# dsteinberg/libcluster

Measured on AMD Instinct MI355X. Metric: E-step data-points/sec (full VBEM iteration: suff-stats + M-step + E-step), higher is better.
Workload: dtype f64

## Files before the change

libcluster_amd/csrc/lc_kernels.h:

```cpp
#pragma once
#include <hip/hip_runtime.h>
#include <cstdint>

namespace lck {

constexpr int RG = 16;

inline int padded_dim(int D) {
  return D <= 16 ? 16 : D <= 32 ? 32 : D <= 48 ? 48 : D <= 64 ? 64 : D <= 80 ? 80 : D <= 96 ? 96 : D <= 112 ? 112 : D <= 128 ? 128 : -1;
}
__host__ __device__ constexpr int lds_row_stride(int DP) { return DP == 16 ? 16 : (DP + 16) % 32 != 16 ? DP + 32 : DP + 16; }
inline int padded_dim_wide(int D) { return D <= 128 ? padded_dim(D) : (D + 63) / 64 * 64; }
constexpr int GW_MAX_DP = 1024;
inline int ntiles(int DP) { int nt = DP / 4; return nt * (nt + 1) / 2; }
inline int pstride(int DP) { return ntiles(DP) * 16 + DP; }
constexpr int WIDE_CHUNK = 256 * 16 + 64;
inline int wide_chunks(int DP) { int np = DP / 64; return np * (np + 1) / 2; }
inline int64_t estep_pstride(int DP, int DC) { return DP > 128 ? (int64_t)wide_chunks(DP) * WIDE_CHUNK : (int64_t)pstride(DC); }
inline int64_t estep_pstride(int DP) { return estep_pstride(DP, DP); }
inline int estep_active_width(int D, int DP) {
  if (DP < 32 || DP > 128) return DP;
  const int g = DP <= 48 ? 4 : 8, lo = DP <= 48 ? DP - 12 : DP - 8;
  const int dc = (D + g - 1) / g * g;
  return dc < DP ? (dc < lo ? lo : dc) : DP;
// ... 54 lines not shown
  int64_t nrg;
  const int* rginfo;
  int64_t nrows;
  const double* params;
  const double* ctab;
  int K;
  double* qZ;
  int64_t ldq;
  double* partial;
  bool want_ll;
  int grid;
  int ngroups = 1;
  int yshare = 0;
};
constexpr int FUSED_CT_CAP = 1024;
inline int64_t fused_record(int DP, int K) { return (int64_t)K * (1 + DP + (int64_t)DP * DP) + 1 + K; }
bool fused_eligible(int DP, int K);
int fused_plan(int DP, int64_t nrg, int K);
hipError_t launch_fused(const FusedLaunch& a, hipStream_t stream);

struct SSItem {
  int64_t r0, r1;
  int kofs, kcnt;
  int64_t rec0;
};
constexpr int SS_BR = 32;
constexpr double SPECK_TAU = 0x1p-300;
enum SuffstatRoute { SS_PER_CLUSTER = 0, SS_FEAT = 1, SS_QUAD = 2, SS_WIDE = 3 };
enum SuffstatMode { SS_DENSE = 0, SS_MASKED_DENSE = 1, SS_ZERO_SKIP = 2, SS_WORK_LIST = 3 };
struct SuffstatPlan {
  SuffstatRoute route;
  int nchunks;
  int64_t chunk_rows;
  int extra, klast0, KR;
  int clusters_per_block;
  const char* name;
};
SuffstatPlan suffstat_plan(int DP, int DC, int64_t NP, int K, SuffstatMode mode);
struct SuffstatLaunch {
  int DP;
  int DC = 0;
  const double* X;
  int64_t NP;
  const double* qZ;
  int64_t ldq;
  int K;
  SuffstatMode mode = SS_DENSE;
  const int* rginfo;
  const unsigned char* smask;
  double* partial;
  int nchunks = 0, KR = 0;
  int64_t chunk_rows = 0;
  const SSItem* items = nullptr;
  const int* klist = nullptr;
  int nitems = 0, skip_listed = 0;
  int speck_skip = 0;
  int nslice = 1;
  int slice0 = 0, rs = 1, klast0 = 0, nklast = 0;
  int64_t ldx = 0;
  int DPW = 0, colA = 0, colB = 0;
};
hipError_t launch_suffstat(const SuffstatLaunch& a, const SuffstatPlan& p, hipStream_t stream);

constexpr int SPECK_PROBE_STEPS = 4096;
constexpr int64_t SPECK_PROBE_MIN_ROWS = 4096;
hipError_t launch_speck_probe(const double* qZ, int64_t ldq, int K, int64_t NP, int* active, int64_t* pairs, hipStream_t stream,
                              int64_t* rows = nullptr);
inline bool speck_probe_says_skip(int64_t active, int64_t pairs) { return pairs > 0 && 4 * (pairs - active) >= pairs; }
bool speck_probe_says_lists(int64_t single, int64_t rows);

struct SsListLayout {
  int nq;
  bool wide;
  size_t ent_off;
  size_t bytes;
};
inline SsListLayout ss_list_layout(int nchunks, int64_t chunk_rows, int K) {
  SsListLayout l{(K + 3) / 4, chunk_rows > 65536, 0, 0};
  l.ent_off = ((size_t)nchunks * l.nq * sizeof(int) + 15) / 16 * 16;
  l.bytes = l.ent_off + (size_t)nchunks * l.nq * (size_t)chunk_rows * (l.wide ? 4 : 2);
  return l;
}
bool suffstat_list_instance(int DP, int DC);
bool speck_lists_enabled();
hipError_t launch_suffstat_list_build(const SuffstatLaunch& a, const SuffstatPlan& p, void* lists, size_t bytes, hipStream_t stream);
hipError_t launch_suffstat_lists(const SuffstatLaunch& a, const SuffstatPlan& p, void* lists, size_t bytes, hipStream_t stream);
hipError_t launch_suffstat_list_build_masks(const SuffstatLaunch& a, const SuffstatPlan& p, const unsigned short* qmask, int64_t nrg,
                                            void* lists, size_t bytes, hipStream_t stream);
hipError_t launch_suffstat_lists_masks(const SuffstatLaunch& a, const SuffstatPlan& p, const unsigned short* qmask, int64_t nrg,
                                       void* lists, size_t bytes, hipStream_t stream);
hipError_t launch_speck_probe_masks(const unsigned short* qmask, int64_t nrg, int K, int64_t NP, int* active, int64_t* pairs,
                                    hipStream_t stream, int64_t* rows = nullptr);
hipError_t launch_qmask_from_qz(const double* qZ, int64_t ldq, int K, int64_t nrg, unsigned short* qmask, hipStream_t stream);
int speck_skip_mode();

__host__ __device__ constexpr int ft_offdiag(int DC) { return (DC / 4) * (DC / 4 - 1) / 2; }
__host__ __device__ constexpr int ft_features(int DC) { return 16 * ft_offdiag(DC) + 10 * (DC / 4) + DC + 1; }
__host__ __device__ constexpr int ft_tiles(int DC) { return (ft_features(DC) + 15) / 16; }
enum FtKind { FT_PRODUCT = 0, FT_LINEAR = 1, FT_COUNT = 2, FT_SPARE = 3 };
struct FtFeature {
  int u, w, kind;
};
__host__ __device__ __attribute__((always_inline)) constexpr FtFeature ft_feature_rest(int DC, int one, int g) {
  const int ndiag = 10 * (DC / 4);
  if (g < ndiag) {
    const int b = 4 * (g / 10), e = g % 10;
    const int i = e < 4 ? 0 : e < 7 ? 1 : e < 9 ? 2 : 3, i0 = e < 4 ? 0 : e < 7 ? 4 : e < 9 ? 7 : 9;
    return {b + i, b + i + (e - i0), FT_PRODUCT};
  }
  g -= ndiag;
  if (g < DC) return {g, one, FT_LINEAR};
  return {one, one, g == DC ? FT_COUNT : FT_SPARE};
}
__host__ __device__ __attribute__((always_inline)) constexpr FtFeature ft_feature(int DC, int one, int f) {
  const int noff = 16 * ft_offdiag(DC);
  if (f < noff) {
    const int p = f / 16, r = f % 16;
    int ja = 1;
    while ((ja + 1) * ja / 2 <= p) ++ja;
    return {4 * (p - ja * (ja - 1) / 2) + (r & 3), 4 * ja + (r >> 2), FT_PRODUCT};
  }
  return ft_feature_rest(DC, one, f - noff);
}
#ifndef LC_FT_WAVES64
#define LC_FT_WAVES64 8
#endif
#ifndef LC_FT_WAVES128
#define LC_FT_WAVES128 8
#endif
__host__ __device__ constexpr int ft_waves(int DP) { return DP == 64 ? LC_FT_WAVES64 : DP == 128 ? LC_FT_WAVES128 : DP > 64 ? 8 : 4; }
__host__ __device__ constexpr int ft_tpw_max(int DP, int NQ) {
  const int t = (NQ >= 8 && DP > 64 && DP < 128 ? 64 : 72) / NQ;
  return t < 14 ? t : 14;
}
__host__ __device__ constexpr int ft_nslice(int DP, int DC, int NQ) {
  return (ft_tiles(DC) + ft_waves(DP) * ft_tpw_max(DP, NQ) - 1) / (ft_waves(DP) * ft_tpw_max(DP, NQ));
}
__host__ __device__ constexpr int ft_tpw(int DP, int DC, int NQ) {
  return (ft_tiles(DC) + ft_waves(DP) * ft_nslice(DP, DC, NQ) - 1) / (ft_waves(DP) * ft_nslice(DP, DC, NQ));
}
__host__ __device__ __attribute__((always_inline)) constexpr void ft_deal(int DP, int DC, int NQ, int slice, int wave, int* t0, int* nt) {
  const int tiles = ft_tiles(DC), nsl = ft_nslice(DP, DC, NQ);
  if (ft_waves(DP) == 8) {
    const int ns = 4 * nsl, s = slice * 4 + (wave & 3), l = tiles / ns, r = tiles % ns;
    const int load = l + (s < r ? 1 : 0), first = s * l + (s < r ? s : r);
    *t0 = first + (wave < 4 ? 0 : (load + 1) / 2);
    *nt = wave < 4 ? (load + 1) / 2 : load / 2;
  } else {
    const int tpw = ft_tpw(DP, DC, NQ), t = (slice * 4 + wave) * tpw;
    *t0 = t;
    *nt = tiles - t < tpw ? (tiles - t > 0 ? tiles - t : 0) : tpw;
  }
}
__host__ __device__ constexpr int ftl_tpw(int DC) { return ((ft_tiles(DC) + 3) / 4 + 1) / 2; }
__host__ __device__ __attribute__((always_inline)) constexpr void ft_deal_one(int DC, int wave, int* t0, int* nt) {
  const int tiles = ft_tiles(DC), s = wave & 3, l = tiles / 4, r = tiles % 4;
  const int load = l + (s < r ? 1 : 0), first = s * l + (s < r ? s : r);
  *t0 = first + (wave < 4 ? 0 : (load + 1) / 2);
  *nt = wave < 4 ? (load + 1) / 2 : load / 2;
}
#ifndef LC_FTL_SHARED
#define LC_FTL_SHARED 1
#endif
__host__ __device__ constexpr bool ftl_shared(int DC) { return LC_FTL_SHARED != 0 && DC == 64; }
__host__ __device__ constexpr int ftl_paired(int DC) { return ftl_shared(DC) ? DC / 4 - 1 : 0; }
__host__ __device__ constexpr int ftl_split(int DC) { return ftl_shared(DC) ? DC / 8 : 0; }
struct FtlFeature {
  int u, w, kind;
  int shared;
};
__host__ __device__ __attribute__((always_inline)) constexpr FtlFeature ftl_feature(int DC, int one, int wave, int t, int l16) {
  if (!ftl_shared(DC)) {
    int t0 = 0, nt = 0;
    ft_deal_one(DC, wave, &t0, &nt);
    if (t >= nt) return {one, one, FT_SPARE, -1};
    const FtFeature f = ft_feature(DC, one, 16 * (t0 + t) + l16);
    return {f.u, f.w, f.kind, -1};
  }
  const int nb = DC / 4, S = ftl_split(DC), P = ftl_paired(DC);
  if (t < P) {
    const int second = t >= S ? 1 : 0, a = wave + second * S, o = (a + 1 + t - second * S) % nb;
    return {4 * o + (l16 & 3), 4 * a + (l16 >> 2), FT_PRODUCT, second};
  }
  const FtFeature f = ft_feature_rest(DC, one, 16 * (2 * wave + t - P) + l16);
  return {f.u, f.w, f.kind, -1};
}
__host__ __device__ constexpr int ftl_nw(int DC) { return ftl_shared(DC) ? 2 + ftl_tpw(DC) - ftl_paired(DC) : ftl_tpw(DC); }
__host__ __device__ constexpr int ftl_wi(int DC, int t) {
  return !ftl_shared(DC) ? t : t < ftl_split(DC) ? 0 : t < ftl_paired(DC) ? 1 : 2 + t - ftl_paired(DC);
}
static_assert(!ftl_shared(64) || (ftl_tpw(64) == ftl_paired(64) + 2 && 16 * 2 * 8 >= ft_features(64) - 16 * ft_offdiag(64)),
              "shared deal: 8 waves of two stars and two free tiles");

__host__ __device__ constexpr int ft_nt_min(int DP, int DC, int NQ) {
  int m = ft_tpw(DP, DC, NQ);
  for (int sl = 0; sl < ft_nslice(DP, DC, NQ); ++sl)
    for (int w = 0; w < ft_waves(DP); ++w) {
      int t0 = 0, nt = 0;
      ft_deal(DP, DC, NQ, sl, w, &t0, &nt);
      m = nt < m ? nt : m;
    }
  return m;
}

hipError_t launch_fold_extra(double* rec, int64_t SS, int K, int klast0, int extra, hipStream_t stream);
hipError_t launch_reduce_records(const double* partial, int64_t n, int K, const int* kptr, const int* krec, double* out,
                                 hipStream_t stream);

constexpr int REDUCE_TMP_ELEMS = 512;
hipError_t launch_reduce_partials(const double* partial, int nparts, int64_t n, double* out, hipStream_t stream,
                                  double* tmp = nullptr);
hipError_t launch_group_colsum(const double* qZ, int64_t ldq, int K, const int64_t* goff, int J, double* out,
                               hipStream_t stream, double* tmp = nullptr, int64_t rows = 0);
hipError_t launch_fill_qz(double* qZ, int64_t ldq, int K, const int* rginfo, int64_t nrows, int64_t nrg, double value,
                          hipStream_t stream);
struct DiagEstepLaunch {
  int DP, D;
  const double* X;
  int64_t nrg;
  const int* rginfo;
  int64_t nrows;
  const double* params;
  int mode = 0;
  const double* ctab;
  int K;
  double* qZ;
  int64_t ldq;
  double* fz_part;
  double* ll_part;
  int raw = 0;
  const double* wt = nullptr;
  const double* mu = nullptr;
  const double* constk = nullptr;
  int ngroups = 1;
  double* sink = nullptr;
};
constexpr int EDM_CT_CAP = 1024;
inline int64_t estep_diag_grid(int64_t nrg) { return (nrg * RG + 63) / 64; }
int64_t estep_diag_mfma_weights(int DP, int K, int mode);
enum DiagEstepInstance { EDI_NONE = 0, EDI_GENERIC = 1, EDI_PLAIN = 2, EDI_TABLED = 3, EDI_ONEGROUP = 4 };
struct DiagEstepPlan {
  bool ok;
  bool mfma;
  int mode;
  int64_t grid;
  size_t lds_bytes;
  const char* name;
  bool wide;
  int KT;
  bool REG;
  int NT;
  bool QUAD;
  int R, KTM;
  int instance;
  int64_t nslots;
  int per_cu;
  int64_t block_cap;
};
DiagEstepPlan estep_diag_plan(const DiagEstepLaunch& a);
hipError_t launch_estep_diag(const DiagEstepLaunch& a, hipStream_t stream);
double estep_diag_centre(int D, int DP, int K, int mode, const double* a, const double* w2, double* mu);
void estep_diag_pack(int D, int DP, int K, int mode, const double* a, const double* w2, const double* w1, const double* mu,
                     double* constk, double* wt, int64_t nw);

struct DiagStatLaunch {
  int DP;
  const double* X;
  int64_t NP;
  const double* qZ;
  int64_t ldq;
  int K;
  const int* rginfo;
  const unsigned char* smask;
  double* partial;
  int nchunks;
// ... 209 lines not shown
```

libcluster_amd/csrc/lc_kernels_suffstat.hip:

```cpp
#include "lc_device.hpp"

#ifndef LC_SS_FEAT_MINK_ACTIVE
#define LC_SS_FEAT_MINK_ACTIVE 5
#endif
#ifndef LC_SS_FEAT_WIDTHS
#define LC_SS_FEAT_WIDTHS(DP) ((DP) >= 32 && (DP) <= 128)
#endif

namespace lck {

template <int NB>
struct SSAcc { static constexpr int N = NB * 3 + NB * (NB - 1) / 2 * 4; };

template <int NB>
__host__ __device__ constexpr bool ss_in_half(int half, int jbp, int jb) {
  if (half == 0) return true;
  const bool first = NB == 8   ? (jbp < 5 || (jbp == 5 && jb < 3))
                     : NB == 7 ? (jbp < 4 || (jbp == 4 && jb < 4))
                     : NB == 6 ? (jbp < 4 || (jbp == 4 && jb < 1))
                               : (jbp == 1 || jbp == 2);
  return first == (half == 1);
}
template <int PAN>
constexpr int ss_batch_rows() { return PAN == 2 ? 24 : SS_BR; }
// ... 1191 lines not shown
#pragma unroll
        for (int t = 0; t < NT; ++t) acc[t] = mfma4(qc, pp[t], acc[t]);
        __builtin_amdgcn_sched_barrier(0);
      } else {
        __builtin_amdgcn_sched_barrier(0);
#pragma unroll
        for (int t = 0; t < NT; ++t) {
          acc[t] = mfma4(qc, pp[t], acc[t]);
          if (st + 1 < BR / 4 && t < SPREAD) {
#pragma unroll
            for (int r = t * NRD / SPREAD; r < (t + 1) * NRD / SPREAD; ++r) {
              const int what = ftl_read(DC, r);
              if (what == NT)
                qa = pq[QO + (st + 1) * 4 * QLD];
              else if (what >= 0)
                uf[what] = pu[what][XO + (st + 1) * 4 * LD];
              else
                wf[-1 - what] = pw[-1 - what][XO + (st + 1) * 4 * LD];
            }
          }
          __builtin_amdgcn_sched_barrier(0);
        }
      }
    }
  };
  if constexpr (LATE) {
    for (int p0 = 0; p0 < len; p0 += 2 * BR) {
      gload();
      iload(p0 + 2 * BR);
      batch(std::integral_constant<int, 0>{});
      lstore(1);
      __syncthreads();
      if (p0 + BR >= len) break;
      gload();
      iload(p0 + 3 * BR);
      batch(std::integral_constant<int, 1>{});
      lstore(0);
      __syncthreads();
    }
  } else {
    for (int p0 = 0; p0 < len; p0 += 2 * BR) {
      const bool more1 = p0 + BR < len, more2 = p0 + 2 * BR < len;
      if (more1) {
        gload();
        iload(p0 + 2 * BR);
      }
      batch(std::integral_constant<int, 0>{});
      if (more1) lstore(1);
      __syncthreads();
      if (!more1) break;
      if (more2) {
        gload();
        iload(p0 + 3 * BR);
      }
      batch(std::integral_constant<int, 1>{});
      if (more2) lstore(0);
      __syncthreads();
    }
  }

  const int64_t SS = 1 + (int64_t)DP + (int64_t)DP * DP;
  int wv = wave;
  asm volatile("" : "+v"(wv));
  const int kk = 4 * quad + hi;
  if (kk >= a.K) return;
  double* out = a.partial + ((int64_t)chunk * a.KR + kk) * SS;
#pragma unroll
  for (int t = 0; t < NT; ++t) {
    const FtlFeature f = ftl_feature(DC, ONE, wv, t, lo2 + 4 * blk);
    if (f.kind == FT_SPARE) continue;
    const double v = acc[t];
    if (f.kind == FT_PRODUCT) {
      double* S = out + 1 + DP;
      S[(int64_t)f.u * DP + f.w] = v;
      S[(int64_t)f.w * DP + f.u] = v;
    } else if (f.kind == FT_LINEAR) {
      out[1 + f.u] = v;
    } else {
      out[0] = v;
    }
  }
}

static hipError_t ss_list_check(const SuffstatLaunch& a, const SuffstatPlan& p, const void* lists, size_t bytes, SsListLayout* lay) {
  if (a.K <= 0 || p.nchunks <= 0 || !lists || !a.qZ || !a.X) return hipErrorInvalidValue;
  if (p.route != SS_FEAT || a.mode != SS_DENSE || a.smask || a.items || p.extra != 0) return hipErrorInvalidValue;
  if (a.nchunks != p.nchunks || a.chunk_rows != p.chunk_rows || a.KR != p.KR || a.KR != a.K) return hipErrorInvalidValue;
  if (!suffstat_list_instance(a.DP, a.DC)) return hipErrorInvalidValue;
  if (a.chunk_rows < 4 || a.chunk_rows % 4 || a.chunk_rows > (int64_t)1 << 30 || (int64_t)a.nchunks * a.chunk_rows < a.NP) return hipErrorInvalidValue;
  *lay = ss_list_layout(a.nchunks, a.chunk_rows, a.K);
  if ((int64_t)a.nchunks * lay->nq > (int64_t)1 << 30 || bytes < lay->bytes) return hipErrorInvalidValue;
  return hipSuccess;
}
hipError_t launch_suffstat_list_build(const SuffstatLaunch& a, const SuffstatPlan& p, void* lists, size_t bytes, hipStream_t stream) {
  SsListLayout lay;
  if (hipError_t e = ss_list_check(a, p, lists, bytes, &lay); e != hipSuccess) return e;
  int* lens = static_cast<int*>(lists);
  void* ent = static_cast<char*>(lists) + lay.ent_off;
  if (lay.wide)
    hipLaunchKernelGGL(ss_list_build_kernel<unsigned>, dim3((unsigned)a.nchunks), dim3(256), 0, stream, a.qZ, a.ldq, a.K, a.NP,
                       a.chunk_rows, lay.nq, lens, static_cast<unsigned*>(ent));
  else
    hipLaunchKernelGGL(ss_list_build_kernel<unsigned short>, dim3((unsigned)a.nchunks), dim3(256), 0, stream, a.qZ, a.ldq, a.K, a.NP,
                       a.chunk_rows, lay.nq, lens, static_cast<unsigned short*>(ent));
  return hipGetLastError();
}
template <int DP, int DC, typename IT>
static hipError_t launch_ss_list_i(const SuffstatLaunch& a, const SsListLayout& lay, const void* lists, hipStream_t stream) {
  constexpr int BR = LC_FTL_BR;
  const size_t shmem = (size_t)(2 * BR * lds_row_stride(DP) + 2 * BR * 4) * sizeof(double);
  auto kern = suffstat_list_kernel<DP, DC, IT>;
  static LdsGrant grant;
  if (hipError_t e = grant_dynamic_lds(reinterpret_cast<const void*>(kern), shmem, grant); e != hipSuccess) return e;
  hipLaunchKernelGGL(kern, dim3((unsigned)(a.nchunks * lay.nq)), dim3(512), shmem, stream, a, static_cast<const int*>(lists),
                     reinterpret_cast<const IT*>(static_cast<const char*>(lists) + lay.ent_off), lay.nq);
  return hipGetLastError();
}
hipError_t launch_suffstat_lists(const SuffstatLaunch& a, const SuffstatPlan& p, void* lists, size_t bytes, hipStream_t stream) {
  SsListLayout lay;
  if (hipError_t e = ss_list_check(a, p, lists, bytes, &lay); e != hipSuccess) return e;
  if (hipError_t e = launch_suffstat_list_build(a, p, lists, bytes, stream); e != hipSuccess) return e;
  const bool narrow = a.DC == 56;
  if (lay.wide) return narrow ? launch_ss_list_i<64, 56, unsigned>(a, lay, lists, stream) : launch_ss_list_i<64, 64, unsigned>(a, lay, lists, stream);
  return narrow ? launch_ss_list_i<64, 56, unsigned short>(a, lay, lists, stream)
                : launch_ss_list_i<64, 64, unsigned short>(a, lay, lists, stream);
}

template <typename IT>
__global__ void __launch_bounds__(256) ss_list_build_masks_kernel(const unsigned short* __restrict__ qmask, int64_t nrg, int64_t NP,
                                                                   int64_t chunk_rows, int nq, int* __restrict__ lens, IT* __restrict__ ent) {
  __shared__ int wcnt[2][4];
  const int chunk = blockIdx.x / nq, c = blockIdx.x % nq, tid = threadIdx.x, lane = tid & 63, wave = tid >> 6;
  const int64_t r0 = (int64_t)chunk * chunk_rows;
  const int64_t r1 = (r0 + chunk_rows) < NP ? (r0 + chunk_rows) : NP;
  if (r0 >= r1) {
    if (tid == 0) lens[blockIdx.x] = 0;
    return;
  }
  const unsigned short* mq = qmask + (int64_t)c * nrg;
  IT* seg = ent + (int64_t)blockIdx.x * chunk_rows;
  int base = 0, par = 0;
  for (int64_t t0 = r0; t0 < r1; t0 += 4096, par ^= 1) {
    const int64_t row = t0 + 16 * tid;
    unsigned m = 0;
    if (row < r1) {
      const int64_t w = row >> 4;
      const unsigned sh = (unsigned)(row & 15);
      const unsigned lo = mq[w], hi = sh != 0 && w + 1 < nrg ? mq[w + 1] : 0u;
      m = ((lo | (hi << 16)) >> sh) & 0xffffu;
      if (r1 - row < 16) m &= (1u << (unsigned)(r1 - row)) - 1u;
    }
    const int cnt = __popc(m);
    int inc = cnt;
#pragma unroll
    for (int d = 1; d < 64; d <<= 1) {
      const int up = __shfl_up(inc, d);
      if (lane >= d) inc += up;
    }
    if (lane == 63) wcnt[par][wave] = inc;
    __syncthreads();
    int before = 0, tot = 0;
#pragma unroll
    for (int w = 0; w < 4; ++w) {
      const int n = wcnt[par][w];
      before += w < wave ? n : 0;
      tot += n;
    }
    int at = base + before + inc - cnt;
    while (m) {
      const int i = __ffs((int)m) - 1;
      m &= m - 1;
      seg[at++] = (IT)(row - r0 + i);
    }
    base += tot;
  }
  if (tid == 0) lens[blockIdx.x] = base;
}
__global__ void __launch_bounds__(256) qmask_from_qz_kernel(const double* __restrict__ qZ, int64_t ldq, int K, int64_t nrg,
                                                             unsigned short* __restrict__ qmask) {
  const int64_t row = (int64_t)blockIdx.x * 256 + threadIdx.x;
  const int c = blockIdx.y, lane = threadIdx.x & 63;
  bool keep = false;
  if (row < nrg * RG) {
#pragma unroll
    for (int i = 0; i < 4; ++i) {
      const int k = 4 * c + i;
      if (k < K && speck_keeps(qZ[(int64_t)k * ldq + row])) keep = true;
    }
  }
  const unsigned long long b = __ballot(keep);
  if ((lane & 15) == 0 && row < nrg * RG) qmask[(int64_t)c * nrg + (row >> 4)] = (unsigned short)((b >> lane) & 0xffffull);
}
hipError_t launch_qmask_from_qz(const double* qZ, int64_t ldq, int K, int64_t nrg, unsigned short* qmask, hipStream_t stream) {
  if (!qZ || !qmask || K < 1 || nrg < 1 || ldq < nrg * RG || (K + 3) / 4 > 65535) return hipErrorInvalidValue;
  hipLaunchKernelGGL(qmask_from_qz_kernel, dim3((unsigned)((nrg * RG + 255) / 256), (unsigned)((K + 3) / 4)), dim3(256), 0, stream, qZ, ldq,
                     K, nrg, qmask);
  return hipGetLastError();
}
hipError_t launch_suffstat_list_build_masks(const SuffstatLaunch& a, const SuffstatPlan& p, const unsigned short* qmask, int64_t nrg,
                                            void* lists, size_t bytes, hipStream_t stream) {
  SsListLayout lay;
  if (hipError_t e = ss_list_check(a, p, lists, bytes, &lay); e != hipSuccess) return e;
  if (!qmask || nrg * RG < a.NP) return hipErrorInvalidValue;
  int* lens = static_cast<int*>(lists);
  void* ent = static_cast<char*>(lists) + lay.ent_off;
  const dim3 grid((unsigned)(a.nchunks * lay.nq));
  if (lay.wide)
    hipLaunchKernelGGL(ss_list_build_masks_kernel<unsigned>, grid, dim3(256), 0, stream, qmask, nrg, a.NP, a.chunk_rows, lay.nq, lens,
                       static_cast<unsigned*>(ent));
  else
    hipLaunchKernelGGL(ss_list_build_masks_kernel<unsigned short>, grid, dim3(256), 0, stream, qmask, nrg, a.NP, a.chunk_rows, lay.nq, lens,
                       static_cast<unsigned short*>(ent));
  return hipGetLastError();
}
hipError_t launch_suffstat_lists_masks(const SuffstatLaunch& a, const SuffstatPlan& p, const unsigned short* qmask, int64_t nrg,
                                       void* lists, size_t bytes, hipStream_t stream) {
  SsListLayout lay;
  if (hipError_t e = launch_suffstat_list_build_masks(a, p, qmask, nrg, lists, bytes, stream); e != hipSuccess) return e;
  if (hipError_t e = ss_list_check(a, p, lists, bytes, &lay); e != hipSuccess) return e;
  const bool narrow = a.DC == 56;
  if (lay.wide) return narrow ? launch_ss_list_i<64, 56, unsigned>(a, lay, lists, stream) : launch_ss_list_i<64, 64, unsigned>(a, lay, lists, stream);
  return narrow ? launch_ss_list_i<64, 56, unsigned short>(a, lay, lists, stream)
                : launch_ss_list_i<64, 64, unsigned short>(a, lay, lists, stream);
}

struct SqItem {
  int kind, ia, ja;
};
__host__ __device__ constexpr int sq_items(int DC) { return (DC / 4) * (DC / 4 + 1) / 2 + DC / 4 + 1; }
__host__ __device__ constexpr SqItem sq_item(int DC, int n) {
  for (int ja = 0; ja < DC / 4; ++ja) {
    if (n <= ja) return SqItem{0, n, ja};
    n -= ja + 1;
    if (n == 0) return SqItem{1, 0, ja};
    n -= 1;
  }
  return SqItem{2, 0, 0};
}
__host__ __device__ constexpr int sq_part_lo(int DC, int NPART, int p) { return (sq_items(DC) * p + NPART - 1) / NPART; }
__host__ __device__ constexpr int sq_part_max(int DC, int NPART) {
  int m = 0;
  for (int p = 0; p < NPART; ++p) {
    const int n = sq_part_lo(DC, NPART, p + 1) - sq_part_lo(DC, NPART, p);
    m = n > m ? n : m;
  }
  return m;
}
constexpr int SQ_BR = 32, SQ_QLD = 18;
inline int sq_npart(int DP, int K) {
  const int nq = (K + 3) / 4;
  if (DP > 48) return 4;
  return nq == 2 ? 2 : nq == 4 ? (DP <= 32 ? 1 : 2) : 4;
}
inline int sq_nslice(int DP, int K) { return (((K + 3) / 4) * sq_npart(DP, K) + 3) / 4; }
inline bool ss_quad_eligible(int DP, int K) {
  static const int mode = test_switch("LC_SS_QUAD") ? atoi(test_switch("LC_SS_QUAD")) : -1;
  if (mode == 0 || DP < 32 || DP > 64 || K < 1 || K > 16) return false;
  if (mode == 1) return true;
  return K >= 3;
}
template <int DP, int DC, int NPART>
__global__ void __launch_bounds__(256, 2) suffstat_quad_kernel(SuffstatLaunch a) {
  static_assert(DC % 4 == 0 && DC <= DP && DC > DP - 16, "active width");
  constexpr int NT = DC / 4, BR = SQ_BR, LD = lds_row_stride(DP), QLD = SQ_QLD, XBUF = BR * LD, QBUF = BR * QLD, NTHR = 256;
  constexpr int NACC = sq_part_max(DC, NPART);
  extern __shared__ __attribute__((aligned(16))) double lds[];
  double* xbuf = lds;
  double* qbuf = lds + 2 * XBUF;
  const int tid = threadIdx.x, lane = tid & 63, wave = tid >> 6;
  const int hi = lane >> 4, blk = (lane >> 2) & 3, lo2 = lane & 3;
  const int K = a.K, NQ = (K + 3) / 4;
  int chunk, slice;
  {
    const int nslice = a.nslice, nchunks = a.nchunks, b = blockIdx.x, full = (nchunks / 8) * 8;
    if (b < full * nslice) {
      const int xcd = b & 7, seq = b >> 3;
      chunk = (seq / nslice) * 8 + xcd;
      slice = seq % nslice;
    } else {
      const int t = b - full * nslice;
      chunk = full + t / nslice;
      slice = t % nslice;
    }
  }
  const int64_t r0 = (int64_t)chunk * a.chunk_rows;
  const int64_t r1 = (r0 + a.chunk_rows) < a.NP ? (r0 + a.chunk_rows) : a.NP;
  const int unit = slice * 4 + wave, quad = unit / NPART, part = unit % NPART;
  const bool busy = quad < NQ;

  constexpr int TPR = DP / 2, NV2 = BR * TPR, NPRE = (NV2 + NTHR - 1) / NTHR;
  double pre[NPRE][2], qpre[4];
  const int qcl = tid % 16, qrq = tid / 16;
  const bool qthr = qrq < BR / 4;
  auto gload = [&](int64_t b0) {
#pragma unroll
    for (int i = 0; i < NPRE; ++i) {
      const int idx = tid + i * NTHR;
      const int row = idx / TPR, c2 = idx % TPR;
      double2 v = make_double2(0.0, 0.0);
      if (row < BR && b0 + row < r1) v = *reinterpret_cast<const double2*>(a.X + (b0 + row) * DP + 2 * c2);
      pre[i][0] = v.x;
      pre[i][1] = v.y;
    }
    const int64_t qrow = b0 + 4 * qrq;
#pragma unroll
    for (int i = 0; i < 4; ++i) qpre[i] = 0.0;
// ... 400 lines not shown
```

libcluster_amd/csrc/lc_testhooks.hip:

```cpp
#include <algorithm>
#include <cstdio>
#include <vector>

#include "lc_device.hpp"
#include "lc_predict.hpp"

namespace {

using lck::RG;
typedef long long i64;

class Scope {
 public:
  ~Scope() {
    for (auto& b : bufs_)
      if (b.d) (void)hipFree(b.d);
  }
  template <typename T>
  T* in(const T* h, size_t n) { return static_cast<T*>(add(const_cast<T*>(h), n * sizeof(T), false, true)); }
  template <typename T>
  T* io(T* h, size_t n) { return static_cast<T*>(add(h, n * sizeof(T), true, true)); }
  template <typename T>
  T* out(T* h, size_t n) { return static_cast<T*>(add(h, n * sizeof(T), true, false)); }
  template <typename T>
// ... 656 lines not shown
      if (klist[t] < 0 || klist[t] >= K) return -1;
    std::vector<char> used((size_t)nrec, 0);
    std::vector<std::vector<int>> recs((size_t)K);
    for (int i = 0; i < nitems; ++i) {
      if (r0[i] < 0 || r0[i] > r1[i] || r1[i] > NP || r0[i] % RG || r1[i] % RG) return -1;
      if (kcnt[i] < 1 || kcnt[i] > p.clusters_per_block || kofs[i] < 0 || kofs[i] > nklist - kcnt[i]) return -1;
      if (rec0[i] < 0 || rec0[i] > nrec - kcnt[i]) return -1;
      for (int t = 0; t < kcnt[i]; ++t) {
        if (used[(size_t)(rec0[i] + t)]) return -1;
        used[(size_t)(rec0[i] + t)] = 1;
        recs[(size_t)klist[kofs[i] + t]].push_back((int)(rec0[i] + t));
      }
      items.push_back(lck::SSItem{r0[i], r1[i], kofs[i], kcnt[i], rec0[i]});
    }
    kptr.assign((size_t)K + 1, 0);
    for (int k = 0; k < K; ++k) {
      krec.insert(krec.end(), recs[(size_t)k].begin(), recs[(size_t)k].end());
      kptr[(size_t)k + 1] = (int)krec.size();
    }
  }
  if (npartial < nrec * SS) return -1;
  Scope s;
  lck::SuffstatLaunch a{};
  a.DP = DP;
  a.DC = DC;
  a.X = s.in(X, (size_t)NP * DP);
  a.NP = NP;
  a.qZ = s.in(qZ, (size_t)K * (size_t)ldq);
  a.ldq = ldq;
  a.K = K;
  a.mode = m;
  a.rginfo = masked ? s.in(rginfo, (size_t)(NP / RG)) : nullptr;
  a.smask = masked ? s.in(smask, (size_t)J * K) : nullptr;
  a.partial = s.io(partial, (size_t)npartial);
  a.nchunks = p.nchunks;
  a.KR = p.KR;
  a.chunk_rows = p.chunk_rows;
  a.speck_skip = speck_skip < 0 ? (p.route == lck::SS_FEAT ? lck::speck_skip_mode() : 0) : speck_skip;
  const int* dkptr = nullptr;
  const int* dkrec = nullptr;
  if (listed) {
    a.items = s.in(items.data(), items.size());
    a.klist = s.in(klist, (size_t)nklist);
    a.nitems = nitems;
    a.skip_listed = skip_listed ? 1 : 0;
    if (fold) {
      dkptr = s.in(kptr.data(), kptr.size());
      dkrec = s.in(krec.data(), krec.size());
    }
  }
  double* dfold = fold ? s.io(folded, (size_t)nfolded) : nullptr;
  double* ext = fold && !listed && p.extra > 0 ? s.scratch<double>((size_t)p.KR * (size_t)SS) : nullptr;
  if (!s.ok()) return s.finish(hipSuccess);
  hipError_t e = lck::launch_suffstat(a, p, nullptr);
  if (e == hipSuccess && fold) {
    if (listed) {
      e = lck::launch_reduce_records(a.partial, SS, K, dkptr, dkrec, dfold, nullptr);
    } else if (p.extra > 0) {
      e = lck::launch_reduce_partials(a.partial, p.nchunks, (i64)p.KR * SS, ext, nullptr);
      if (e == hipSuccess) e = lck::launch_fold_extra(ext, SS, K, p.klast0, p.extra, nullptr);
      if (e == hipSuccess) e = hipMemcpyAsync(dfold, ext, (size_t)K * (size_t)SS * sizeof(double), hipMemcpyDeviceToDevice, nullptr);
    } else {
      e = lck::launch_reduce_partials(a.partial, p.nchunks, (i64)K * SS, dfold, nullptr);
    }
  }
  return s.finish(e);
}
LC_HOOK lc_test_suffstat(const double* X, int DP, int DC, i64 NP, const double* qZ, int K, i64 ldq, int mode, const int* rginfo,
                         const unsigned char* smask, int J, int nitems, const i64* r0, const i64* r1, const int* kofs, const int* kcnt,
                         const i64* rec0, const int* klist, int nklist, int nrec_listed, int skip_listed, double* partial, i64 npartial,
                         int fold, double* folded, i64 nfolded, i64* plan_out) {
  return test_suffstat(X, DP, DC, NP, qZ, K, ldq, mode, rginfo, smask, J, nitems, r0, r1, kofs, kcnt, rec0, klist, nklist, nrec_listed,
                       skip_listed, partial, npartial, fold, folded, nfolded, plan_out, -1);
}
LC_HOOK lcx_test_suffstat_speck(const double* X, int DP, int DC, i64 NP, const double* qZ, int K, i64 ldq, int mode, const int* rginfo,
                                const unsigned char* smask, int J, int nitems, const i64* r0, const i64* r1, const int* kofs,
                                const int* kcnt, const i64* rec0, const int* klist, int nklist, int nrec_listed, int skip_listed,
                               double* partial, i64 npartial, int fold, double* folded, i64 nfolded, i64* plan_out, int speck_skip) {
  if (speck_skip < 0 || speck_skip > 2) return -1;
  return test_suffstat(X, DP, DC, NP, qZ, K, ldq, mode, rginfo, smask, J, nitems, r0, r1, kofs, kcnt, rec0, klist, nklist, nrec_listed,
                       skip_listed, partial, npartial, fold, folded, nfolded, plan_out, speck_skip);
}

LC_HOOK lcx_test_suffstat_lists(const double* X, int DP, int DC, i64 NP, const double* qZ, int K, i64 ldq, int sums, double* partial,
                                i64 npartial, int fold, double* folded, i64 nfolded, i64* plan_out, int* lens_out, i64 nlens, int* ent_out,
                                i64 nent) {
  if (!X || !qZ || !partial || !plan_out || !lens_out || !ent_out || K < 1 || K > 4096 || !gw_width_ok(DP, DC)) return -1;
  if (NP < RG || NP % RG || NP > HOT_MAX_NRG * RG || ldq < NP || ldq % 2) return -1;
  const i64 SS = lck::stat_stride(DP);
  if (fold && (!sums || !folded || nfolded < (i64)K * SS)) return -1;
  const lck::SuffstatPlan p = lck::suffstat_plan(DP, DC, NP, K, lck::SS_DENSE);
  plan_out[0] = p.route, plan_out[1] = p.nchunks, plan_out[2] = p.chunk_rows, plan_out[3] = p.extra, plan_out[4] = p.klast0;
  plan_out[5] = p.KR, plan_out[6] = p.clusters_per_block;
  if (p.nchunks < 1 || p.chunk_rows < lck::SS_BR || p.chunk_rows % lck::SS_BR || (i64)p.nchunks * p.chunk_rows < NP) return -1;
  const lck::SsListLayout lay = lck::ss_list_layout(p.nchunks, p.chunk_rows, K);
  const i64 nseg = (i64)p.nchunks * lay.nq;
  if (npartial < (i64)p.nchunks * p.KR * SS || nlens < nseg || nent < nseg * p.chunk_rows) return -1;
  Scope s;
  lck::SuffstatLaunch a{};
  a.DP = DP;
  a.DC = DC;
  a.X = s.in(X, (size_t)NP * DP);
  a.NP = NP;
  a.qZ = s.in(qZ, (size_t)K * (size_t)ldq);
  a.ldq = ldq;
  a.K = K;
  a.mode = lck::SS_DENSE;
  a.rginfo = nullptr;
  a.smask = nullptr;
  a.partial = s.io(partial, (size_t)npartial);
  a.nchunks = p.nchunks;
  a.KR = p.KR;
  a.chunk_rows = p.chunk_rows;
  unsigned char* lists = s.scratch<unsigned char>(lay.bytes);
  double* dfold = fold ? s.io(folded, (size_t)nfolded) : nullptr;
  if (!s.ok()) return s.finish(hipSuccess);
  hipError_t e = hipMemset(lists, 0xff, lay.bytes);
  if (e == hipSuccess)
    e = sums ? lck::launch_suffstat_lists(a, p, lists, lay.bytes, nullptr) : lck::launch_suffstat_list_build(a, p, lists, lay.bytes, nullptr);
  if (e == hipSuccess && fold) e = lck::launch_reduce_partials(a.partial, p.nchunks, (i64)K * SS, dfold, nullptr);
  const int rc = s.finish(e);
  if (rc != 0) return rc;
  std::vector<unsigned char> raw(lay.bytes);
  if (hipMemcpy(raw.data(), lists, lay.bytes, hipMemcpyDeviceToHost) != hipSuccess) return -1;
  const int* lens = reinterpret_cast<const int*>(raw.data());
  for (i64 g = 0; g < nseg; ++g)
    if (lens[g] < 0 || lens[g] > p.chunk_rows) return -2;
  for (i64 g = 0; g < nseg; ++g) {
    lens_out[g] = lens[g];
    for (int i = 0; i < lens[g]; ++i) {
      const size_t at = (size_t)g * (size_t)p.chunk_rows + (size_t)i;
      ent_out[at] = lay.wide ? (int)reinterpret_cast<const unsigned*>(raw.data() + lay.ent_off)[at]
                             : (int)reinterpret_cast<const unsigned short*>(raw.data() + lay.ent_off)[at];
    }
  }
  return 0;
}

LC_HOOK lcx_test_estep_masks(const double* X, int DP, int DC, i64 nrg, const double* params, const double* ctab, int J, const int* rginfo,
                             i64 nrows, int K, double* qZ, int Kbuf, i64 ldq, double* fz_part, i64 nfz, double* ll_part, i64 nll,
                             unsigned short* qmask, i64 nmask, int* emits) {
  if (!X || !params || !ctab || !qZ || !fz_part || !emits || K < 1 || K > 4096 || Kbuf < K || Kbuf > 8192 || J < 1 || J > (1 << 20)) return -1;
  if (nrg < 1 || nrg > HOT_MAX_NRG || ldq < nrg * RG || !gw_width_ok(DP, DC)) return -1;
  if (rginfo ? !rginfo_ok(rginfo, nrg, J) : (J != 1 || nrows < 0 || nrows > nrg * RG)) return -1;
  if (qmask && nmask < (i64)((K + 3) / 4) * nrg) return -1;
  lck::EstepLaunch a{};
  a.DP = DP;
  a.DC = DC;
  a.K = K;
  a.nrg = nrg;
  a.nrows = nrows;
  a.ldq = ldq;
  const lck::EstepPlan p = lck::estep_plan(a);
  if (!p.ok || p.grid < 1 || p.lds_bytes > HOT_LDS_LIMIT) return -1;
  if (nfz < p.grid || (ll_part && nll < p.grid * K)) return -1;
  *emits = p.emits ? 1 : 0;
  Scope s;
  a.X = s.in(X, (size_t)(nrg * RG) * DP);
  a.params = s.in(params, (size_t)K * (size_t)lck::estep_pstride(DP, p.DC));
  a.ctab = s.in(ctab, (size_t)J * K);
  a.rginfo = rginfo ? s.in(rginfo, (size_t)nrg) : nullptr;
  a.qZ = s.io(qZ, (size_t)Kbuf * (size_t)ldq);
  a.fz_part = s.io(fz_part, (size_t)nfz);
  a.ll_part = ll_part ? s.io(ll_part, (size_t)nll) : nullptr;
  a.qmask = qmask ? s.io(qmask, (size_t)nmask) : nullptr;
  if (!s.ok()) return s.finish(hipSuccess);
  return s.finish(lck::launch_estep(a, nullptr));
}

LC_HOOK lcx_test_list_build(int which, const double* qZ, int DC, i64 NP, int K, i64 ldq, const unsigned short* qmask, i64 chunk_rows,
                            i64* out, int* lens_out, i64 nlens, int* ent_out, i64 nent) {
  const int DP = 64;
  if (!qZ || !qmask || !out || !lens_out || !ent_out || K < 1 || K > 4096 || !gw_width_ok(DP, DC)) return -1;
  if (NP < RG || NP % RG || NP > HOT_MAX_NRG * RG || ldq < NP || chunk_rows < 0 || chunk_rows % 4) return -1;
  lck::SuffstatPlan p = lck::suffstat_plan(DP, DC, NP, K, lck::SS_DENSE);
  if (chunk_rows > 0) {
    p.chunk_rows = chunk_rows;
    p.nchunks = (int)((NP + chunk_rows - 1) / chunk_rows);
  }
  if (p.nchunks < 1 || p.chunk_rows < 4 || (i64)p.nchunks * p.chunk_rows < NP) return -1;
  out[0] = p.nchunks, out[1] = p.chunk_rows;
  const lck::SsListLayout lay = lck::ss_list_layout(p.nchunks, p.chunk_rows, K);
  const i64 nseg = (i64)p.nchunks * lay.nq, nrg = NP / RG;
  if (nlens < nseg || nent < nseg * p.chunk_rows) return -1;
  Scope s;
  lck::SuffstatLaunch a{};
  a.DP = DP;
  a.DC = DC;
  a.X = s.scratch<double>(16);
  a.NP = NP;
  a.qZ = s.in(qZ, (size_t)K * (size_t)ldq);
  a.ldq = ldq;
  a.K = K;
  a.mode = lck::SS_DENSE;
  a.nchunks = p.nchunks;
  a.KR = p.KR;
  a.chunk_rows = p.chunk_rows;
  const unsigned short* dmask = s.in(qmask, (size_t)lay.nq * (size_t)nrg);
  unsigned char* lists = s.scratch<unsigned char>(lay.bytes);
  if (!s.ok()) return s.finish(hipSuccess);
  hipError_t e = hipMemset(lists, 0xff, lay.bytes);
  if (e == hipSuccess)
    e = which ? lck::launch_suffstat_list_build_masks(a, p, dmask, nrg, lists, lay.bytes, nullptr)
              : lck::launch_suffstat_list_build(a, p, lists, lay.bytes, nullptr);
  const int rc = s.finish(e);
  if (rc != 0) return rc;
  std::vector<unsigned char> raw(lay.bytes);
  if (hipMemcpy(raw.data(), lists, lay.bytes, hipMemcpyDeviceToHost) != hipSuccess) return -1;
  const int* lens = reinterpret_cast<const int*>(raw.data());
  for (i64 g = 0; g < nseg; ++g)
    if (lens[g] < 0 || lens[g] > p.chunk_rows) return -2;
  for (i64 g = 0; g < nseg; ++g) {
    lens_out[g] = lens[g];
    for (int i = 0; i < lens[g]; ++i) {
      const size_t at = (size_t)g * (size_t)p.chunk_rows + (size_t)i;
      ent_out[at] = lay.wide ? (int)reinterpret_cast<const unsigned*>(raw.data() + lay.ent_off)[at]
                             : (int)reinterpret_cast<const unsigned short*>(raw.data() + lay.ent_off)[at];
    }
  }
  return 0;
}

LC_HOOK lcx_test_speck_probe(int which, const double* qZ, i64 ldq, int K, i64 NP, const unsigned short* qmask, i64* out) {
  if (!qZ || !qmask || !out || K < 1 || K > 4096 || NP < RG || NP % RG || NP > HOT_MAX_NRG * RG || ldq < NP || ldq % 2) return -1;
  const i64 nrg = NP / RG;
  Scope s;
  const double* dq = s.in(qZ, (size_t)K * (size_t)ldq);
  const unsigned short* dm = s.in(qmask, (size_t)((K + 3) / 4) * (size_t)nrg);
  int* act = s.scratch<int>(2);
  if (!s.ok()) return s.finish(hipSuccess);
  int64_t pairs = 0, rows = 0;
  const hipError_t e = which ? lck::launch_speck_probe_masks(dm, nrg, K, NP, act, &pairs, nullptr, &rows)
                             : lck::launch_speck_probe(dq, ldq, K, NP, act, &pairs, nullptr, &rows);
  const int rc = s.finish(e);
  if (rc != 0) return rc;
  int h[2] = {0, 0};
  if (hipMemcpy(h, act, sizeof(h), hipMemcpyDeviceToHost) != hipSuccess) return -1;
  out[0] = h[0], out[1] = h[1], out[2] = pairs, out[3] = rows;
  return 0;
}

LC_HOOK lcx_test_suffstat_list_deal(int DP, int DC, i64* info, int* feat, i64 nfeat) {
  if (!info || !feat || !gw_width_ok(DP, DC) || !lck::suffstat_list_instance(DP, DC)) return -1;
  const int dc = DC ? DC : DP, waves = 8, tiles = lck::ftl_tpw(dc);
  if (nfeat < (i64)waves * tiles * 16 * 4) return -1;
  info[0] = lck::ftl_shared(dc) ? 1 : 0, info[1] = waves, info[2] = tiles, info[3] = lck::ftl_paired(dc), info[4] = lck::ftl_split(dc);
  info[5] = DP;
  for (int v = 0; v < waves; ++v)
    for (int t = 0; t < tiles; ++t)
      for (int l = 0; l < 16; ++l) {
        const lck::FtlFeature f = lck::ftl_feature(dc, DP, v, t, l);
        int* o = feat + ((size_t)(v * tiles + t) * 16 + l) * 4;
        o[0] = f.u, o[1] = f.w, o[2] = f.kind, o[3] = f.shared;
      }
  return 0;
}

LC_HOOK lc_test_fused_plan(int DP, i64 nrg, int K, i64* out) {
  if (!out || K < 1 || K > 4096 || nrg < 0 || nrg > HOT_MAX_NRG || DP < 1 || DP > 1024) return -1;
  out[0] = lck::fused_eligible(DP, K) ? 1 : 0;
  out[1] = lck::fused_plan(DP, nrg, K);
  out[2] = lck::current_device_cus();
  out[3] = (i64)lck::fused_record(DP, K);
  return 0;
}
LC_HOOK lc_test_fused(const double* X, int D, i64 nrg, const double* params, const double* ctab, int J, const int* rginfo, i64 nrows,
                      int K, int want_ll, int grid, double* qZ, int Kbuf, i64 ldq, double* partial, i64 npartial, int* grid_used) {
  const int DP = 16;
  if (!X || !params || !ctab || !qZ || !partial || !grid_used || D < 1 || D > DP || K < 1 || Kbuf < K || Kbuf > 8192) return -1;
  if (nrg < 1 || nrg > HOT_MAX_NRG || ldq < nrg * RG || J < 1 || J > (1 << 20) || !lck::fused_eligible(DP, K)) return -1;
  if (rginfo ? !rginfo_ok(rginfo, nrg, J) : (J != 1 || nrows < 0 || nrows > nrg * RG)) return -1;
  const int plan = lck::fused_plan(DP, nrg, K);
  if (plan < 1 || grid < 0 || grid > plan) return -1;
  const int g = grid ? grid : plan;
  if (npartial < (i64)g * lck::fused_record(DP, K)) return -1;
  *grid_used = g;
  Scope s;
  lck::FusedLaunch a{};
  a.DP = DP;
  a.D = D;
  a.X = s.in(X, (size_t)(nrg * RG) * DP);
  a.nrg = nrg;
  a.rginfo = rginfo ? s.in(rginfo, (size_t)nrg) : nullptr;
  a.nrows = nrows;
  a.params = s.in(params, (size_t)K * (size_t)lck::pstride(DP));
  a.ctab = s.in(ctab, (size_t)J * K);
  a.K = K;
  a.qZ = s.io(qZ, (size_t)Kbuf * (size_t)ldq);
  a.ldq = ldq;
  a.partial = s.io(partial, (size_t)npartial);
  a.want_ll = want_ll != 0;
  a.grid = g;
  a.ngroups = J;
  if (!s.ok()) return s.finish(hipSuccess);
  return s.finish(lck::launch_fused(a, nullptr));
}

namespace {

bool diag_width_ok(int DP) { return DP >= 16 && (DP <= 128 ? DP % 16 == 0 : (DP % 64 == 0 && DP <= 1024)); }

void diag_estep_plan_out(const lck::DiagEstepPlan& p, i64* out, char* name) {
  out[0] = p.ok ? 1 : 0, out[1] = p.mfma ? 1 : 0, out[2] = p.mode, out[3] = p.grid, out[4] = (i64)p.lds_bytes;
  out[5] = p.wide ? 1 : 0, out[6] = p.KT, out[7] = p.REG ? 1 : 0, out[8] = p.NT, out[9] = p.QUAD ? 1 : 0, out[10] = p.R;
  out[11] = p.KTM, out[12] = p.instance, out[13] = p.nslots, out[14] = p.per_cu, out[15] = p.block_cap;
  if (name) snprintf(name, 32, "%s", p.name ? p.name : "");
}
void diag_stat_plan_out(const lck::DiagStatPlan& p, i64* out, char* name) {
  out[0] = p.ok ? 1 : 0, out[1] = p.nslice, out[2] = p.rsplit, out[3] = p.second, out[4] = p.nblocks, out[5] = p.width;
  out[6] = p.last_width, out[7] = p.BR, out[8] = p.BR_last, out[9] = p.nstage ? 1 : 0, out[10] = p.nstage_last ? 1 : 0;
  out[11] = p.deep ? 1 : 0, out[12] = p.deep_last ? 1 : 0, out[13] = (i64)p.lds_bytes;
  if (name) snprintf(name, 32, "%s", p.name ? p.name : "");
}
constexpr int DIAG_SINK = 256, DIAG_SINK_GUARD = 64;

}

LC_HOOK lc_test_estep_diag_plan(int DP, int K, int mode, i64 nrg, int mfma, int raw, int want_ll, int grouped, int ngroups,
                                i64* out, char* name) {
  if (!out || !name || K < 1 || K > 4096 || nrg < 0 || nrg > HOT_MAX_NRG || DP < 1 || DP > 1024 || mode < 0 || mode > 2 || ngroups < 1)
    return -1;
  static double some;
  static int somei;
  lck::DiagEstepLaunch a{};
  a.DP = DP, a.D = DP, a.K = K, a.mode = mode, a.nrg = nrg, a.raw = raw ? 1 : 0, a.ngroups = ngroups;
  a.wt = mfma ? &some : nullptr;
  a.ll_part = want_ll ? &some : nullptr;
  a.rginfo = grouped ? &somei : nullptr;
  diag_estep_plan_out(lck::estep_diag_plan(a), out, name);
  return 0;
}
LC_HOOK lc_test_estep_diag(const double* X, int DP, i64 nrg, const double* params, int mode, const double* ctab, int J,
                           const int* rginfo, i64 nrows, int K, int raw, const double* wt, i64 nwt, const double* mu,
                           const double* constk, double* qZ, int Kbuf, i64 ldq, double* fz_part, i64 nfz, double* ll_part, i64 nll,
                           double* sink, i64* plan_out, char* name) {
  if (!X || !params || !ctab || !qZ || !fz_part || !plan_out || !name || K < 1 || K > 4096 || Kbuf < K || Kbuf > 8192) return -1;
  if (J < 1 || J > (1 << 20) || mode < 0 || mode > 2 || nrg < 1 || nrg > HOT_MAX_NRG || nrg * RG > ldq) return -1;
  if (!diag_width_ok(DP)) return -1;
  if (rginfo ? !rginfo_ok(rginfo, nrg, J) : (J != 1 || nrows < 0 || nrows > nrg * RG)) return -1;
  if (wt) {
// ... 90 lines not shown
```

Measured before the change: 392.3 million.

## Add column-owner suffstat kernel for DP=64 list path

Adds a new sufficient-statistics kernel for D=64 on the sparse list route. Each cluster gets one wave, and each lane owns a column, accumulating 33 cyclic diagonals of the outer product in registers. Row values are broadcast through LDS and several rows are prefetched in flight, replacing the previous tile-dealt feature kernel. The aim is fewer wasted accumulators and better reuse, at the cost of more per-row LDS round trips and wave barriers, plus mirrored writes for the symmetric output.

Result: faster. 417.1 million (median of 6 runs) (+6.3%).

```diff
diff --git a/libcluster_amd/csrc/lc_kernels.h b/libcluster_amd/csrc/lc_kernels.h
--- a/libcluster_amd/csrc/lc_kernels.h
+++ b/libcluster_amd/csrc/lc_kernels.h
@@ -160,6 +160,7 @@
   return l;
 }
 bool suffstat_list_instance(int DP, int DC);
+bool suffstat_owner_instance(int DP, int DC);
 bool speck_lists_enabled();
 hipError_t launch_suffstat_list_build(const SuffstatLaunch& a, const SuffstatPlan& p, void* lists, size_t bytes, hipStream_t stream);
 hipError_t launch_suffstat_lists(const SuffstatLaunch& a, const SuffstatPlan& p, void* lists, size_t bytes, hipStream_t stream);
@@ -269,6 +270,13 @@
 }
 static_assert(!ftl_shared(64) || (ftl_tpw(64) == ftl_paired(64) + 2 && 16 * 2 * 8 >= ft_features(64) - 16 * ft_offdiag(64)),
               "shared deal: 8 waves of two stars and two free tiles");
+
+constexpr int FTO_DIAGS = 33, FTO_ACCS = 35;
+__host__ __device__ __attribute__((always_inline)) constexpr FtFeature fto_feature(int lane, int t) {
+  if (t < FTO_DIAGS) return {lane, (lane + t) & 63, t == 32 && lane >= 32 ? FT_SPARE : FT_PRODUCT};
+  if (t == FTO_DIAGS) return {lane, 64, FT_LINEAR};
+  return {64, 64, lane == 0 ? FT_COUNT : FT_SPARE};
+}
 
 __host__ __device__ constexpr int ft_nt_min(int DP, int DC, int NQ) {
   int m = ft_tpw(DP, DC, NQ);
diff --git a/libcluster_amd/csrc/lc_kernels_suffstat.hip b/libcluster_amd/csrc/lc_kernels_suffstat.hip
--- a/libcluster_amd/csrc/lc_kernels_suffstat.hip
+++ b/libcluster_amd/csrc/lc_kernels_suffstat.hip
@@ -1297,6 +1297,137 @@
   }
 }
 
+#ifndef LC_FTL_OWNER
+#define LC_FTL_OWNER 1
+#endif
+#ifndef LC_FTO_DEPTH
+#define LC_FTO_DEPTH 4
+#endif
+#ifndef LC_FTO_FUSED
+#define LC_FTO_FUSED 1
+#endif
+bool suffstat_owner_instance(int DP, int DC) { return LC_FTL_OWNER != 0 && DP == 64 && (DC == 0 || DC == 64); }
+template <int DP, int DC, typename IT>
+__global__ void __launch_bounds__(256, 4) suffstat_owner_kernel(SuffstatLaunch a, const int* __restrict__ lens, const IT* __restrict__ ent,
+                                                                 int nq) {
+  static_assert(DP == 64 && DC == 64, "lane w owns column w");
+  constexpr int G = LC_FTO_DEPTH, NSLOT = 2, ND = FTO_DIAGS;
+  static_assert(G >= 1 && G <= 8, "rows in flight");
+  __shared__ double slots[4][NSLOT][2 * DP];
+  const int lane = threadIdx.x & 63, wave = __builtin_amdgcn_readfirstlane((int)(threadIdx.x >> 6));
+  const int chunk = blockIdx.x / nq, quad = blockIdx.x % nq;
+  const int k = 4 * quad + wave;
+  if (k >= a.K) return;
+  const int64_t r0 = (int64_t)chunk * a.chunk_rows;
+  const int64_t rows64 = a.NP - r0 < a.chunk_rows ? a.NP - r0 : a.chunk_rows;
+  const int rows = rows64 > 0 ? (int)rows64 : 0;
+  int len = lens[blockIdx.x];
+  len = len < 0 ? 0 : len > rows ? rows : len;
+  const int nwin = (len + 63) / 64;
+  const IT* li = ent + (int64_t)blockIdx.x * a.chunk_rows;
+  const int64_t rb = rows > 0 ? r0 : 0;
+  const double* qcol = a.qZ + (int64_t)k * a.ldq + rb;
+  const double* xl = a.X + rb * DP + lane;
+  double* slot = &slots[wave][0][lane];
+
+  double acc[ND], lin = 0.0, cnt = 0.0;
+#pragma unroll
+  for (int t = 0; t < ND; ++t) acc[t] = 0.0;
+
+  auto ld_off = [&](int w) {
+    const int p = 64 * w + lane;
+    const int o = p < len ? (int)li[p] : 0;
+    return o < rows ? o : 0;
+  };
+  int widx = -1;
+  unsigned long long mask = 0ull;
+  int cur_off = 0, n1_off = ld_off(0), n2_off = ld_off(1);
+  double cur_q = 0.0, n1_q = qcol[n1_off];
+  auto advance = [&]() {
+    ++widx;
+    cur_off = n1_off, cur_q = n1_q;
+    n1_off = n2_off;
+    n1_q = qcol[n1_off];
+    n2_off = ld_off(widx + 2);
+    mask = __ballot(64 * widx + lane < len && speck_keeps(cur_q));
+  };
+  auto fetch = [&](double(&gx)[G], double(&gq)[G], int& n) {
+    while (mask == 0ull && widx + 1 < nwin) advance();
+    n = 0;
+#pragma unroll
+    for (int i = 0; i < G; ++i) {
+      const bool has = mask != 0ull;
+      const int l = has ? __builtin_ctzll(mask) : 0;
+      mask &= mask - (has ? 1ull : 0ull);
+      const int off = has ? __builtin_amdgcn_readlane(cur_off, l) : 0;
+      gq[i] = readlane_f64(cur_q, l);
+      gx[i] = xl[(int64_t)off * DP];
+      n += has ? 1 : 0;
+    }
+  };
+  auto row = [&](double x, double q, int s) {
+    double* sl = slot + s * 2 * DP;
+    __builtin_amdgcn_fence(__ATOMIC_RELEASE, "wavefront");
+    __builtin_amdgcn_wave_barrier();
+    sl[0] = x;
+    sl[DP] = x;
+    __builtin_amdgcn_fence(__ATOMIC_ACQ_REL, "wavefront");
+    __builtin_amdgcn_wave_barrier();
+    double y[ND];
+    y[0] = x;
+#pragma unroll
+    for (int t = 1; t < ND; ++t) {
+      y[t] = sl[t];
+      asm volatile("" ::: "memory");
+    }
+#pragma unroll
+    for (int t = 0; t < ND; ++t) {
+      const double p = x * y[t];
+#if LC_FTO_FUSED
+      acc[t] = fma(q, p, acc[t]);
+#else
+      acc[t] = __dadd_rn(__dmul_rn(q, p), acc[t]);
+#endif
+    }
+#if LC_FTO_FUSED
+    lin = fma(q, x, lin);
+    cnt = fma(q, 1.0, cnt);
+#else
+    lin = __dadd_rn(__dmul_rn(q, x), lin);
+    cnt = __dadd_rn(q, cnt);
+#endif
+  };
+  auto sum = [&](const double(&gx)[G], const double(&gq)[G], int n) {
+#pragma unroll
+    for (int i = 0; i < G; ++i)
+      if (i < n) row(gx[i], gq[i], i % NSLOT);
+  };
+  double ax[G], aq[G], bx[G], bq[G];
+  int an = 0, bn = 0;
+  fetch(ax, aq, an);
+  while (an > 0) {
+    fetch(bx, bq, bn);
+    sum(ax, aq, an);
+    if (bn == 0) break;
+    fetch(ax, aq, an);
+    sum(bx, bq, bn);
+  }
+
+  const int64_t SS = 1 + (int64_t)DP + (int64_t)DP * DP;
+  double* out = a.partial + ((int64_t)chunk * a.KR + k) * SS;
+  double* S = out + 1 + DP;
+#pragma unroll
+  for (int t = 0; t < ND; ++t) {
+    const FtFeature f = fto_feature(lane, t);
+    if (f.kind == FT_PRODUCT) {
+      S[f.u * DP + f.w] = acc[t];
+      if (t != 0) S[f.w * DP + f.u] = acc[t];
+    }
+  }
+  out[1 + fto_feature(lane, ND).u] = lin;
+  if (fto_feature(lane, ND + 1).kind == FT_COUNT) out[0] = cnt;
+}
+
 static hipError_t ss_list_check(const SuffstatLaunch& a, const SuffstatPlan& p, const void* lists, size_t bytes, SsListLayout* lay) {
   if (a.K <= 0 || p.nchunks <= 0 || !lists || !a.qZ || !a.X) return hipErrorInvalidValue;
   if (p.route != SS_FEAT || a.mode != SS_DENSE || a.smask || a.items || p.extra != 0) return hipErrorInvalidValue;
@@ -1331,14 +1462,22 @@
                      reinterpret_cast<const IT*>(static_cast<const char*>(lists) + lay.ent_off), lay.nq);
   return hipGetLastError();
 }
+template <typename IT>
+static hipError_t launch_ss_owner_i(const SuffstatLaunch& a, const SsListLayout& lay, const void* lists, hipStream_t stream) {
+  hipLaunchKernelGGL((suffstat_owner_kernel<64, 64, IT>), dim3((unsigned)(a.nchunks * lay.nq)), dim3(256), 0, stream, a,
+                     static_cast<const int*>(lists), reinterpret_cast<const IT*>(static_cast<const char*>(lists) + lay.ent_off), lay.nq);
+  return hipGetLastError();
+}
+static hipError_t launch_ss_list_sums(const SuffstatLaunch& a, const SsListLayout& lay, const void* lists, hipStream_t stream) {
+  if (a.DC == 56) return lay.wide ? launch_ss_list_i<64, 56, unsigned>(a, lay, lists, stream) : launch_ss_list_i<64, 56, unsigned short>(a, lay, lists, stream);
+  if (suffstat_owner_instance(a.DP, a.DC)) return lay.wide ? launch_ss_owner_i<unsigned>(a, lay, lists, stream) : launch_ss_owner_i<unsigned short>(a, lay, lists, stream);
+  return lay.wide ? launch_ss_list_i<64, 64, unsigned>(a, lay, lists, stream) : launch_ss_list_i<64, 64, unsigned short>(a, lay, lists, stream);
+}
 hipError_t launch_suffstat_lists(const SuffstatLaunch& a, const SuffstatPlan& p, void* lists, size_t bytes, hipStream_t stream) {
   SsListLayout lay;
   if (hipError_t e = ss_list_check(a, p, lists, bytes, &lay); e != hipSuccess) return e;
   if (hipError_t e = launch_suffstat_list_build(a, p, lists, bytes, stream); e != hipSuccess) return e;
-  const bool narrow = a.DC == 56;
-  if (lay.wide) return narrow ? launch_ss_list_i<64, 56, unsigned>(a, lay, lists, stream) : launch_ss_list_i<64, 64, unsigned>(a, lay, lists, stream);
-  return narrow ? launch_ss_list_i<64, 56, unsigned short>(a, lay, lists, stream)
-                : launch_ss_list_i<64, 64, unsigned short>(a, lay, lists, stream);
+  return launch_ss_list_sums(a, lay, lists, stream);
 }
 
 template <typename IT>
@@ -1433,10 +1572,7 @@
   SsListLayout lay;
   if (hipError_t e = launch_suffstat_list_build_masks(a, p, qmask, nrg, lists, bytes, stream); e != hipSuccess) return e;
   if (hipError_t e = ss_list_check(a, p, lists, bytes, &lay); e != hipSuccess) return e;
-  const bool narrow = a.DC == 56;
-  if (lay.wide) return narrow ? launch_ss_list_i<64, 56, unsigned>(a, lay, lists, stream) : launch_ss_list_i<64, 64, unsigned>(a, lay, lists, stream);
-  return narrow ? launch_ss_list_i<64, 56, unsigned short>(a, lay, lists, stream)
-                : launch_ss_list_i<64, 64, unsigned short>(a, lay, lists, stream);
+  return launch_ss_list_sums(a, lay, lists, stream);
 }
 
 struct SqItem {
diff --git a/libcluster_amd/csrc/lc_testhooks.hip b/libcluster_amd/csrc/lc_testhooks.hip
--- a/libcluster_amd/csrc/lc_testhooks.hip
+++ b/libcluster_amd/csrc/lc_testhooks.hip
@@ -762,14 +762,18 @@
                        skip_listed, partial, npartial, fold, folded, nfolded, plan_out, speck_skip);
 }
 
-LC_HOOK lcx_test_suffstat_lists(const double* X, int DP, int DC, i64 NP, const double* qZ, int K, i64 ldq, int sums, double* partial,
-                                i64 npartial, int fold, double* folded, i64 nfolded, i64* plan_out, int* lens_out, i64 nlens, int* ent_out,
-                                i64 nent) {
+static int test_suffstat_lists(const double* X, int DP, int DC, i64 NP, const double* qZ, int K, i64 ldq, int sums, double* partial,
+                               i64 npartial, int fold, double* folded, i64 nfolded, i64* plan_out, int* lens_out, i64 nlens, int* ent_out,
+                               i64 nent, i64 chunk_rows) {
   if (!X || !qZ || !partial || !plan_out || !lens_out || !ent_out || K < 1 || K > 4096 || !gw_width_ok(DP, DC)) return -1;
-  if (NP < RG || NP % RG || NP > HOT_MAX_NRG * RG || ldq < NP || ldq % 2) return -1;
+  if (NP < RG || NP % RG || NP > HOT_MAX_NRG * RG || ldq < NP || ldq % 2 || chunk_rows < 0 || chunk_rows % lck::SS_BR) return -1;
   const i64 SS = lck::stat_stride(DP);
   if (fold && (!sums || !folded || nfolded < (i64)K * SS)) return -1;
-  const lck::SuffstatPlan p = lck::suffstat_plan(DP, DC, NP, K, lck::SS_DENSE);
+  lck::SuffstatPlan p = lck::suffstat_plan(DP, DC, NP, K, lck::SS_DENSE);
+  if (chunk_rows > 0) {
+    p.chunk_rows = chunk_rows;
+    p.nchunks = (int)((NP + chunk_rows - 1) / chunk_rows);
+  }
   plan_out[0] = p.route, plan_out[1] = p.nchunks, plan_out[2] = p.chunk_rows, plan_out[3] = p.extra, plan_out[4] = p.klast0;
   plan_out[5] = p.KR, plan_out[6] = p.clusters_per_block;
   if (p.nchunks < 1 || p.chunk_rows < lck::SS_BR || p.chunk_rows % lck::SS_BR || (i64)p.nchunks * p.chunk_rows < NP) return -1;
@@ -817,6 +821,20 @@
   return 0;
 }
 
+LC_HOOK lcx_test_suffstat_lists(const double* X, int DP, int DC, i64 NP, const double* qZ, int K, i64 ldq, int sums, double* partial,
+                                i64 npartial, int fold, double* folded, i64 nfolded, i64* plan_out, int* lens_out, i64 nlens, int* ent_out,
+                                i64 nent) {
+  return test_suffstat_lists(X, DP, DC, NP, qZ, K, ldq, sums, partial, npartial, fold, folded, nfolded, plan_out, lens_out, nlens, ent_out,
+                             nent, 0);
+}
+LC_HOOK lcx_test_suffstat_lists_chunked(const double* X, int DP, int DC, i64 NP, const double* qZ, int K, i64 ldq, i64 chunk_rows,
+                                        double* partial, i64 npartial, double* folded, i64 nfolded, i64* plan_out, int* lens_out, i64 nlens,
+                                        int* ent_out, i64 nent) {
+  if (chunk_rows < 1) return -1;
+  return test_suffstat_lists(X, DP, DC, NP, qZ, K, ldq, 1, partial, npartial, 1, folded, nfolded, plan_out, lens_out, nlens, ent_out, nent,
+                             chunk_rows);
+}
+
 LC_HOOK lcx_test_estep_masks(const double* X, int DP, int DC, i64 nrg, const double* params, const double* ctab, int J, const int* rginfo,
                              i64 nrows, int K, double* qZ, int Kbuf, i64 ldq, double* fz_part, i64 nfz, double* ll_part, i64 nll,
                              unsigned short* qmask, i64 nmask, int* emits) {
@@ -936,6 +954,18 @@
   return 0;
 }
 
+LC_HOOK lcx_test_suffstat_owner_deal(i64* info, int* feat, i64 nfeat) {
+  if (!info || !feat || nfeat < (i64)lck::FTO_ACCS * 64 * 3) return -1;
+  info[0] = lck::FTO_DIAGS, info[1] = lck::FTO_ACCS, info[2] = lck::suffstat_owner_instance(64, 64) ? 1 : 0;
+  for (int t = 0; t < lck::FTO_ACCS; ++t)
+    for (int l = 0; l < 64; ++l) {
+      const lck::FtFeature f = lck::fto_feature(l, t);
+      int* o = feat + ((size_t)t * 64 + l) * 3;
+      o[0] = f.u, o[1] = f.w, o[2] = f.kind;
+    }
+  return 0;
+}
+
 LC_HOOK lc_test_fused_plan(int DP, i64 nrg, int K, i64* out) {
   if (!out || K < 1 || K > 4096 || nrg < 0 || nrg > HOT_MAX_NRG || DP < 1 || DP > 1024) return -1;
   out[0] = lck::fused_eligible(DP, K) ? 1 : 0;
```
